# PJLab-ADG/OpenPCSeg

Measured on AMD Instinct MI355X. Metric: LiDAR frames/sec training MinkUNet-34 SemanticKITTI, higher is better.
Workload: dtype f32; 1 GPU; MinkUNet-34 cr1.0 train step, 12 x 120k-pt synthetic SemanticKITTI scans/GPU, fp32; global_batch=12, voxels_per_gpu_batch=1158864, parallelism=dp1, wgrad=fp32

## Files before the change

### include/pcseg_hip.h

```cpp
#ifndef PCSEG_HIP_H_
#define PCSEG_HIP_H_

#include <stddef.h>
#include <stdint.h>

#ifdef __cplusplus
extern "C" {
#endif

#define PCS_OK 0
#define PCS_EINVAL (-1)
#define PCS_EWORKSPACE (-2)
#define PCS_ELAUNCH (-3)
#define PCS_EUNSUPPORTED (-4)

#define PCS_ABI_VERSION 12

int pcs_abi_version(void);
const char *pcs_last_error(void);

int pcs_hash(const int32_t *coords, int64_t n, int64_t *out, void *stream);

int pcs_kernel_hash(const int32_t *coords, int64_t n, const int32_t *offsets, int32_t K,
                    int64_t *out, void *stream);
// ... 233 lines not shown
int pcs_predict_points_f32(const float *logits, int64_t m, int32_t c, const int64_t *inverse, int64_t n,
                           const int64_t *point_offset, const int64_t *row_offset, int32_t n_scenes,
                           const int64_t *labels, float *votes, int64_t *pred, int64_t *hist, int32_t *bad_flag,
                           void *stream);

typedef struct {
  const float *src;
  void *dst;
  int32_t K, A, B;
  int32_t kind;
  int32_t transpose;
  int32_t nctt, nt16, ns;
  int64_t first_block;
} pcs_weight_job;
int64_t pcs_weights_multi_plan(pcs_weight_job *jobs_host, int32_t n_jobs);
int pcs_weights_multi(const pcs_weight_job *jobs_dev, int32_t n_jobs, int64_t total_blocks, void *stream);

int64_t pcs_lovasz_workspace_bytes(int64_t n, int32_t num_class, int32_t has_ignore, int64_t ignore);
int pcs_lovasz_softmax_f32(const float *probas, const int64_t *labels, int64_t n, int32_t num_class, int32_t has_ignore,
                           int64_t ignore, float *loss, float *grad, void *ws, int64_t ws_bytes, void *stream);

void pcs_debug_convh_ws(int32_t mode, int32_t ru, int32_t rs);
void pcs_debug_wgrad_interleave(int32_t mode);

#ifdef __cplusplus
}
#endif
#endif
```

### openpcseg_amd/csrc/conv_wgrad.hip

```cpp
#include "conv_common.h"

using namespace pcs;

namespace {

constexpr int WG_PB = 32;
constexpr int WG_TS = 128 + 16;

struct WgradArgs {
  const float *fa;
  const float *fb;
  const int32_t *pairs;
  const int32_t *koff;
  float *partial;
  int ca, cb, K, a_col, pch;
};

__device__ __forceinline__ void find_split(const int32_t *koff, int K, int pch, int split, int *k_out,
                                           int *beg, int *end) {
  int acc = 0;
  for (int k = 0; k < K; ++k) {
    const int nk = koff[k + 1] - koff[k];
    const int ns = (nk + pch - 1) / pch;
    if (split < acc + ns) {
      const int s = split - acc;
      *k_out = k;
      *beg = koff[k] + s * pch;
      const int e = *beg + pch;
      *end = e < koff[k + 1] ? e : koff[k + 1];
      return;
    }
    acc += ns;
  }
  *k_out = -1; *beg = 0; *end = 0;
}

__device__ __forceinline__ void find_split_wave(const int32_t *koff, int K, int pch, int split, int lane, int *beg,
                                                int *end, int *gsid, int interleave) {
  if (K > 64) {
    int k;
    find_split(koff, K, pch, split, &k, beg, end);
    *gsid = split;
    return;
  }
  const int lo = lane < K ? koff[lane] : 0, hi = lane < K ? koff[lane + 1] : 0;
  const int ns = (hi - lo + pch - 1) / pch;
  int incl = ns;
  for (int o = 1; o < 64; o <<= 1) {
    const int t = __shfl_up(incl, o, 64);
    if (lane >= o) incl += t;
  }
  int src, sidx;
  if (!interleave) {
    const unsigned long long hit = __ballot(split >= incl - ns && split < incl);
    if (!hit) { *beg = 0; *end = 0; *gsid = split; return; }
    src = __ffsll((long long)hit) - 1;
    sidx = split - __shfl(incl - ns, src, 64);
  } else {
    const int total = __shfl(incl, 63, 64);
    if (interleave == 2) {
      const int chunk = (total + 7) >> 3;
      split = (split & 7) * chunk + (split >> 3);
    }
    if (split >= total) { *beg = 0; *end = 0; *gsid = 0; return; }
    int rmax = ns;
    for (int o = 32; o > 0; o >>= 1) { const int t = __shfl_xor(rmax, o, 64); rmax = t > rmax ? t : rmax; }
    auto upto = [&](int r) {
      int c = ns > 0 ? (int)(((long long)r * ns) / rmax) + 1 : 0;
      for (int o = 32; o > 0; o >>= 1) c += __shfl_xor(c, o, 64);
      return c;
    };
    int a = 0, b = rmax - 1;
    while (a < b) {
      const int m = (a + b) >> 1;
      if (upto(m) > split) b = m; else a = m + 1;
    }
    const int r = a;
    const int before = r > 0 ? upto(r - 1) : 0;
    const int s_r = ns > 0 ? (int)(((long long)r * ns) / rmax) : -1;
    const int s_p = (ns > 0 && r > 0) ? (int)(((long long)(r - 1) * ns) / rmax) : -1;
    unsigned long long fresh = __ballot(ns > 0 && s_r != s_p);
    int want = split - before;
    while (want > 0) { fresh &= fresh - 1; --want; }
    src = __ffsll((long long)fresh) - 1;
    sidx = __shfl(s_r, src, 64);
  }
  const int b0 = lo + sidx * pch;
  const int e0 = b0 + pch < hi ? b0 + pch : hi;
  *beg = __shfl(b0, src, 64);
  *end = __shfl(e0, src, 64);
  *gsid = __shfl(incl - ns, src, 64) + sidx;
}

__global__ void __launch_bounds__(256) wgrad_kernel(WgradArgs w) {
  __shared__ __attribute__((aligned(16))) float abuf[WG_PB * WG_TS];
  __shared__ __attribute__((aligned(16))) float bbuf[WG_PB * WG_TS];
  __shared__ int ia[WG_PB], ib[WG_PB];
  __shared__ int sh[3];
  const int tid = threadIdx.x, lane = tid & 63, wid = tid >> 6;
  const int a0 = blockIdx.y * 128, b0 = blockIdx.z * 128;
  const int cat = (w.ca - a0) < 128 ? (w.ca - a0) : 128;
  const int cbt = (w.cb - b0) < 128 ? (w.cb - b0) : 128;
  const int ta_n = (cat + 15) / 16, tb_n = (cbt + 15) / 16;
  if (tid == 0) find_split(w.koff, w.K, w.pch, blockIdx.x, &sh[0], &sh[1], &sh[2]);
  __syncthreads();
  const int beg = sh[1], end = sh[2];
  const int wa = wid >> 1, wb = wid & 1;
  f32x4 acc[4][4];
#pragma unroll
  for (int i = 0; i < 4; ++i)
#pragma unroll
    for (int j = 0; j < 4; ++j) acc[i][j] = (f32x4){0, 0, 0, 0};

  const int capad = ta_n * 16, cbpad = tb_n * 16;
  for (int p0 = beg; p0 < end; p0 += WG_PB) {
    const int np = (end - p0) < WG_PB ? (end - p0) : WG_PB;
    __syncthreads();
    if (tid < WG_PB) {
      int2 p = make_int2(-1, -1);
      if (tid < np) p = reinterpret_cast<const int2 *>(w.pairs)[p0 + tid];
      ia[tid] = w.a_col ? p.y : p.x;
      ib[tid] = w.a_col ? p.x : p.y;
    }
    __syncthreads();
    for (int e = tid; e < WG_PB * capad; e += 256) {
      const int r = e / capad, c = e % capad;
      abuf[r * WG_TS + c] = (r < np && c < cat) ? w.fa[(int64_t)ia[r] * w.ca + a0 + c] : 0.f;
// ... 28 lines not shown
        }
      }
    }
  }
  float *out = w.partial + (int64_t)blockIdx.x * w.ca * w.cb;
  const int g = lane >> 4, l15 = lane & 15;
#pragma unroll
  for (int i = 0; i < 4; ++i) {
    const int ta = wa + 2 * i;
    if (ta >= ta_n) continue;
#pragma unroll
    for (int j = 0; j < 4; ++j) {
      const int tb = wb + 2 * j;
      if (tb >= tb_n) continue;
#pragma unroll
      for (int r = 0; r < 4; ++r) {
        const int ra = ta * 16 + g * 4 + r, cbv = tb * 16 + l15;
        if (ra < cat && cbv < cbt) out[(int64_t)(a0 + ra) * w.cb + b0 + cbv] = acc[i][j][r];
      }
    }
  }
}

__global__ void __launch_bounds__(256) wgrad_reduce_kernel(const float *__restrict__ partial,
                                                           const int32_t *__restrict__ koff,
                                                           int K, int pch, int64_t cc,
                                                           float *__restrict__ gW) {
  const int k = blockIdx.y;
  __shared__ int sh[2];
  if (threadIdx.x == 0) {
    int acc = 0;
    for (int q = 0; q < k; ++q) acc += (koff[q + 1] - koff[q] + pch - 1) / pch;
    sh[0] = acc;
    sh[1] = (koff[k + 1] - koff[k] + pch - 1) / pch;
  }
  __syncthreads();
  const int base = sh[0], ns = sh[1];
  for (int64_t e = (int64_t)blockIdx.x * blockDim.x + threadIdx.x; e < cc;
       e += (int64_t)gridDim.x * blockDim.x) {
    float s = 0.f;
    for (int q = 0; q < ns; ++q) s += partial[(int64_t)(base + q) * cc + e];
    gW[(int64_t)k * cc + e] = s;
  }
}

__global__ void __launch_bounds__(256) wgrad_reduce4_kernel(const float *__restrict__ partial,
                                                            const int32_t *__restrict__ koff,
                                                            int K, int pch, int64_t cc,
                                                            float *__restrict__ gW) {
  const int k = blockIdx.y;
  __shared__ int sh[2];
  __shared__ float4 red[16][16];
  if (threadIdx.x < 64) {
    const int lane = threadIdx.x;
    int acc = 0, mine = 0;
    if (K <= 64) {
      const int nsq = lane < K ? (koff[lane + 1] - koff[lane] + pch - 1) / pch : 0;
      int incl = nsq;
      for (int o = 1; o < 64; o <<= 1) {
        const int t = __shfl_up(incl, o, 64);
        if (lane >= o) incl += t;
      }
      acc = __shfl(incl - nsq, k, 64);
      mine = __shfl(nsq, k, 64);
    } else {
      for (int q = 0; q < k; ++q) acc += (koff[q + 1] - koff[q] + pch - 1) / pch;
      mine = (koff[k + 1] - koff[k] + pch - 1) / pch;
    }
    if (lane == 0) { sh[0] = acc; sh[1] = mine; }
  }
  __syncthreads();
  const int base = sh[0], ns = sh[1];
  const int et = threadIdx.x & 15, ql = threadIdx.x >> 4;
  const int64_t e = ((int64_t)blockIdx.x * 16 + et) * 4;
  const bool ok = e < cc;
  const float *p = partial + (int64_t)base * cc + (ok ? e : 0);
  float4 s0 = {0, 0, 0, 0}, s1 = s0, s2 = s0, s3 = s0;
  int q = ql;
  for (; q + 48 < ns; q += 64) {
    const float4 v0 = *reinterpret_cast<const float4 *>(p + (int64_t)q * cc);
    const float4 v1 = *reinterpret_cast<const float4 *>(p + (int64_t)(q + 16) * cc);
    const float4 v2 = *reinterpret_cast<const float4 *>(p + (int64_t)(q + 32) * cc);
    const float4 v3 = *reinterpret_cast<const float4 *>(p + (int64_t)(q + 48) * cc);
    s0.x += v0.x; s0.y += v0.y; s0.z += v0.z; s0.w += v0.w;
    s1.x += v1.x; s1.y += v1.y; s1.z += v1.z; s1.w += v1.w;
    s2.x += v2.x; s2.y += v2.y; s2.z += v2.z; s2.w += v2.w;
    s3.x += v3.x; s3.y += v3.y; s3.z += v3.z; s3.w += v3.w;
  }
  for (; q < ns; q += 16) {
    const float4 v0 = *reinterpret_cast<const float4 *>(p + (int64_t)q * cc);
    s0.x += v0.x; s0.y += v0.y; s0.z += v0.z; s0.w += v0.w;
  }
  s0.x += s1.x + (s2.x + s3.x); s0.y += s1.y + (s2.y + s3.y);
  s0.z += s1.z + (s2.z + s3.z); s0.w += s1.w + (s2.w + s3.w);
  red[ql][et] = s0;
  __syncthreads();
  if (ql == 0 && ok) {
    float4 t = red[0][et];
#pragma unroll
    for (int j = 1; j < 16; ++j) {
      const float4 v = red[j][et];
      t.x += v.x; t.y += v.y; t.z += v.z; t.w += v.w;
    }
    *reinterpret_cast<float4 *>(gW + (int64_t)k * cc + e) = t;
  }
}

struct Wgrad2Args {
  const void *fa;
  const void *fb;
  const int32_t *pairs;
  const int32_t *koff;
  float *partial;
  int ca, cb, K, a_col, pch, nbg;
  int interleave;
};

__host__ __device__ inline int wg_ngroups(int c) { return (c + 63) / 64; }
__host__ __device__ inline int wg_gwidth(int c) {
  const int per = (c + wg_ngroups(c) - 1) / wg_ngroups(c);
  return (per + 15) / 16 * 16;
}

template <int W> struct WVec;
template <> struct WVec<64> { using T = float4; static constexpr int N = 4; };
template <> struct WVec<48> { using T = float3; static constexpr int N = 3; };
template <> struct WVec<32> { using T = float2; static constexpr int N = 2; };
template <> struct WVec<16> { using T = float;  static constexpr int N = 1; };
__device__ __forceinline__ float wcomp(const float4 &v, int i) { return i == 0 ? v.x : (i == 1 ? v.y : (i == 2 ? v.z : v.w)); }
__device__ __forceinline__ float wcomp(const float3 &v, int i) { return i == 0 ? v.x : (i == 1 ? v.y : v.z); }
__device__ __forceinline__ float wcomp(const float2 &v, int i) { return i == 0 ? v.x : v.y; }
__device__ __forceinline__ float wcomp(const float &v, int) { return v; }

template <typename V, int N> __device__ __forceinline__ V wload(Fp32, const void *base, int64_t elem) {
  return *reinterpret_cast<const V *>(reinterpret_cast<const float *>(base) + elem);
}
template <typename V, int N, typename HT> __device__ __forceinline__ V wload(HT, const void *base, int64_t elem) {
  const uint16_t *p = reinterpret_cast<const uint16_t *>(base) + elem;
// ... 90 lines not shown
#else
    acc[0][0][1] += wcomp(b1s.a[0], 0) + wcomp(b1s.a[1], 0) + wcomp(b1s.a[2], 0) + wcomp(b1s.a[3], 0) + wcomp(b1s.b[0], 0) + wcomp(b1s.b[1], 0) + wcomp(b1s.b[2], 0) + wcomp(b1s.b[3], 0);
#endif
    __builtin_amdgcn_sched_barrier(0);
  }
#pragma unroll
  for (int f = 0; f < NA; ++f) {
#pragma unroll
    for (int r = 0; r < 4; ++r) {
      const int row = a0 + NA * (4 * g + r) + f;
      if (row < w.ca && bok) {
        float *d = out + (int64_t)row * w.cb + bc;
#pragma unroll
        for (int h = 0; h < NB; ++h) d[h] = acc[f][h][r];
      }
    }
  }
}

template <typename ET>
__global__ void __launch_bounds__(256, 3) wgrad2_kernel(Wgrad2Args w) {
  const int tid = threadIdx.x, lane = tid & 63, wid = tid >> 6;
  int beg, end, gsid;
  find_split_wave(w.koff, w.K, w.pch, blockIdx.x, lane, &beg, &end, &gsid, w.interleave);
  const int nag = wg_ngroups(w.ca);
  const int nsb = (w.nbg + 1) >> 1;
  const int sa = blockIdx.y / nsb, sb = blockIdx.y - sa * nsb;
  const int ag = 2 * sa + (wid >> 1), bg = 2 * sb + (wid & 1);
  if (beg >= end || ag >= nag || bg >= w.nbg) return;
  const int aw = wg_gwidth(w.ca), bw = wg_gwidth(w.cb);
  float *out = w.partial + (int64_t)gsid * w.ca * w.cb;
  const int a0 = aw * ag, b0 = bw * bg;
#define PCS_WG_CASE(A, B) if (aw == A && bw == B) { wgrad_block<A, B, ET>(w, a0, b0, beg, end, out, lane); return; }
  PCS_WG_CASE(64, 64) PCS_WG_CASE(64, 48) PCS_WG_CASE(64, 32) PCS_WG_CASE(64, 16)
  PCS_WG_CASE(48, 64) PCS_WG_CASE(48, 48) PCS_WG_CASE(48, 32) PCS_WG_CASE(48, 16)
  PCS_WG_CASE(32, 64) PCS_WG_CASE(32, 48) PCS_WG_CASE(32, 32) PCS_WG_CASE(32, 16)
  PCS_WG_CASE(16, 64) PCS_WG_CASE(16, 48) PCS_WG_CASE(16, 32) PCS_WG_CASE(16, 16)
#undef PCS_WG_CASE
}

constexpr int W3_PB = 32;
constexpr int W3_ROW = 128;

typedef __bf16 w3_bf16x2 __attribute__((ext_vector_type(2)));
typedef float w3_f32x2 __attribute__((ext_vector_type(2)));
typedef __bf16 w3_bf16x8 __attribute__((ext_vector_type(8)));
typedef _Float16 w3_f16x8 __attribute__((ext_vector_type(8)));

struct Wgrad3Args {
  const void *fa;
  const void *fb;
  const int32_t *pairs;
  const int32_t *koff;
  float *partial;
  int ca, cb, K, a_col, pch;
  int aw, bw, nag, nbg, nsb;
  int interleave;
  int nsy = 1;
};

template <typename ET> struct W3Mode;
template <> struct W3Mode<Fp32> { static constexpr int PLANES = 3; using MT = Bf16; };
template <> struct W3Mode<Bf16> { static constexpr int PLANES = 1; using MT = Bf16; };
template <> struct W3Mode<Fp16> { static constexpr int PLANES = 1; using MT = Fp16; };

__device__ __forceinline__ f32x4 w3_mfma(Bf16, const uint4 &a, const uint4 &b, f32x4 c) {
  return __builtin_amdgcn_mfma_f32_16x16x32_bf16(__builtin_bit_cast(w3_bf16x8, a), __builtin_bit_cast(w3_bf16x8, b), c, 0, 0, 0);
}
__device__ __forceinline__ f32x4 w3_mfma(Fp16, const uint4 &a, const uint4 &b, f32x4 c) {
  return __builtin_amdgcn_mfma_f32_16x16x32_f16(__builtin_bit_cast(w3_f16x8, a), __builtin_bit_cast(w3_f16x8, b), c, 0, 0, 0);
}

__device__ __forceinline__ void w3_split(float x, float y, uint32_t &hi, uint32_t &mid, uint32_t &lo) {
  const w3_f32x2 v = {x, y};
  const w3_bf16x2 h = __builtin_convertvector(v, w3_bf16x2);
  const w3_f32x2 r1 = v - __builtin_convertvector(h, w3_f32x2);
  const w3_bf16x2 m = __builtin_convertvector(r1, w3_bf16x2);
  const w3_f32x2 r2 = r1 - __builtin_convertvector(m, w3_f32x2);
  const w3_bf16x2 l = __builtin_convertvector(r2, w3_bf16x2);
  hi = __builtin_bit_cast(uint32_t, h); mid = __builtin_bit_cast(uint32_t, m); lo = __builtin_bit_cast(uint32_t, l);
}

template <typename ET, int NA, int NB, int NT = 256, int ROW = W3_ROW>
__global__ void __launch_bounds__(NT, NT == 256 ? (W3Mode<ET>::PLANES == 1 ? 3 : 2) : 4) wgrad3_kernel(Wgrad3Args w) {
  constexpr int PL = W3Mode<ET>::PLANES;
  using MT = typename W3Mode<ET>::MT;
  constexpr bool F32IN = std::is_same<ET, Fp32>::value;
  constexpr int NBUF = PL == 1 ? 2 : 1;
  constexpr int IMG = PL * 2 * W3_PB * ROW;
  __shared__ __attribute__((aligned(16))) uint16_t lds[NBUF * IMG];
  const int tid = threadIdx.x, lane = tid & 63, wid = tid >> 6;
  const int g = lane >> 4, l15 = lane & 15;
  int beg, end, gsid;
  int bx = blockIdx.x, by = blockIdx.y;
  if (w.interleave == 2 && w.nsy > 1) {
    const int slot = bx >> 3;
    by = slot % w.nsy;
    bx = ((slot / w.nsy) << 3) | (bx & 7);
  }
  find_split_wave(w.koff, w.K, w.pch, bx, lane, &beg, &end, &gsid, w.interleave);
  if (beg >= end) return;
  const int sa = by / w.nsb, sb = by - sa * w.nsb;
  const int a_base = 2 * sa * w.aw, b_base = 2 * sb * w.bw;
  const int a_stage = (w.ca - a_base) < 2 * w.aw ? (w.ca - a_base) : 2 * w.aw;
  const int b_stage = (w.cb - b_base) < 2 * w.bw ? (w.cb - b_base) : 2 * w.bw;
  const int ag = 2 * sa + (wid >> 1), bg = 2 * sb + (wid & 1);
  const bool active = ag < w.nag && bg < w.nbg;
  const int aoff = (wid >> 1) * w.aw, boff = (wid & 1) * w.bw;

  f32x4 acc[NA][NB];
#pragma unroll
  for (int i = 0; i < NA; ++i)
#pragma unroll
    for (int j = 0; j < NB; ++j) acc[i][j] = (f32x4){0, 0, 0, 0};

  constexpr int CPP = F32IN ? 4 : 8;
  constexpr int PPR = ROW / CPP;
  constexpr int PIECES = (W3_PB / 2) * PPR / NT;
  static_assert(PIECES >= 1 && (W3_PB / 2) * PPR % NT == 0, "staging items must divide over the threads");
  uint32_t *ldw = reinterpret_cast<uint32_t *>(lds);
  constexpr int IMGW = IMG / 2;
  constexpr int OPW = (W3_PB / 2) * ROW;
  auto wpos = [](int q, int ch) { return q * ROW + ((((ch >> 4) ^ (q >> 2)) & (ROW / 16 - 1)) << 4) + (ch & 15); };
// ... 116 lines not shown
      __syncthreads();
      if (more) stage(0);
      __syncthreads();
    }
  }
  if (!active) return;
  const int a0 = a_base + aoff, b0 = b_base + boff;
  float *out = w.partial + (int64_t)gsid * w.ca * w.cb;
#pragma unroll
  for (int i = 0; i < NA; ++i)
#pragma unroll
    for (int r = 0; r < 4; ++r) {
      const int row = a0 + 16 * i + 4 * g + r;
      if (row < w.ca) {
#pragma unroll
        for (int j = 0; j < NB; ++j) {
          const int col = b0 + 16 * j + l15;
          if (col < w.cb) out[(int64_t)row * w.cb + col] = acc[i][j][r];
        }
      }
    }
}

struct WgradEnv { int wgrad3, thin, target, interleave; };
const WgradEnv &wgrad_env() {
  auto num = [](const char *v, int dflt) { return v ? atoi(v) : dflt; };
  static const WgradEnv env = {num(getenv("PCS_WGRAD3"), 1),
                               num(getenv("PCS_WGRAD3_THIN"), 1),
                               num(getenv("PCS_WGRAD_TARGET"), 0),
                               num(getenv("PCS_WGRAD_INTERLEAVE"), -1)};
  return env;
}

int g_wgrad_interleave = -1;
enum class WgradFamily { generic, wgrad2, wgrad3, wgrad3_thin };
struct WgradPlan { WgradFamily family; int pch, ns, interleave; dim3 grid; };

int wgrad_splits(const int32_t *koff_host, int K, int pch) {
  int64_t ns = 0;
  for (int k = 0; k < K; ++k) ns += ceil_div((int64_t)koff_host[k + 1] - koff_host[k], pch);
  return (int)ns;
}

WgradPlan wgrad_route(const int32_t *koff_host, int K, int ca, int cb, int dtype, bool force_split, bool operands_aligned,
                      int use3 = wgrad_env().wgrad3, bool count = true) {
  const WgradEnv &env = wgrad_env();
  const bool half = dtype != 0;
  const int nag = wg_ngroups(ca), nbg = wg_ngroups(cb);
  WgradPlan p;
  const bool thin = use3 >= 1 && env.thin && half && ca % 16 == 0 && cb % 16 == 0 && ca <= 64 && cb <= 64 && ca >= 32 && cb >= 32 &&
                    operands_aligned;
  const bool vec = (ca % 4 == 0) && (cb % 4 == 0) && operands_aligned;
  const int cgran = half ? 8 : 4;
  const bool want3 = !half ? (use3 == 2 || force_split) : (use3 >= 1 && (use3 == 2 || nag * nbg >= 4));
  p.family = thin ? WgradFamily::wgrad3_thin
                  : (vec && want3 && ca % cgran == 0 && cb % cgran == 0) ? WgradFamily::wgrad3
                                                                         : (vec ? WgradFamily::wgrad2 : WgradFamily::generic);
  const int nbq = (nag * nbg + 3) / 4;
  const int64_t P = koff_host[K] - koff_host[0];
  int64_t target = (env.target > 0 ? env.target : (nbq >= 4 ? (half ? 2048 : 3072) : 1536)) / nbq;
  if (thin) target *= 4;
  if (target < K) target = K;
  p.pch = (int)ceil_div(P > 0 ? P : 1, target);
  p.pch = (int)(ceil_div(p.pch, 32) * 32);
  if (p.pch < 64) p.pch = 64;
  p.ns = count ? wgrad_splits(koff_host, K, p.pch) : 0;
  p.interleave = g_wgrad_interleave >= 0 ? g_wgrad_interleave : (env.interleave >= 0 ? env.interleave : (half ? 2 : 0));
  const unsigned nx = (unsigned)(p.interleave == 2 ? 8 * ((p.ns + 7) / 8) : p.ns), nsy = (unsigned)(((nag + 1) / 2) * ((nbg + 1) / 2));
  if (p.family == WgradFamily::generic) p.grid = dim3((unsigned)p.ns, (unsigned)ceil_div(ca, 128), (unsigned)ceil_div(cb, 128));
  else if (p.family == WgradFamily::wgrad2) p.grid = dim3(nx, nsy);
  else p.grid = p.interleave == 2 ? dim3(nx * nsy, 1u) : dim3((unsigned)p.ns, nsy);
  return p;
}

template <typename Args>
Args wgrad_args(const void *fa, const void *fb, const int32_t *pairs, const int32_t *koff_dev, void *ws, int ca, int cb, int K,
                int a_col, int pch) {
  Args w;
  w.fa = static_cast<decltype(w.fa)>(fa); w.fb = static_cast<decltype(w.fb)>(fb); w.pairs = pairs; w.koff = koff_dev;
  w.partial = reinterpret_cast<float *>(ws);
  w.ca = ca; w.cb = cb; w.K = K; w.a_col = a_col; w.pch = pch;
  return w;
}

template <typename ET, int NT, int ROW>
int launch_wgrad3(const Wgrad3Args &w, dim3 grid, hipStream_t st, const char *what) {
  const int na = w.aw / 16, nb = w.bw / 16;
#define PCS_W3_CASE(A, B) if constexpr (NT == 256 || (A >= 2 && B >= 2)) if (na == A && nb == B) { hipLaunchKernelGGL((wgrad3_kernel<ET, A, B, NT, ROW>), grid, dim3(NT), 0, st, w); return check_launch(what); }
  PCS_W3_CASE(4, 4) PCS_W3_CASE(4, 3) PCS_W3_CASE(4, 2) PCS_W3_CASE(4, 1)
  PCS_W3_CASE(3, 4) PCS_W3_CASE(3, 3) PCS_W3_CASE(3, 2) PCS_W3_CASE(3, 1)
  PCS_W3_CASE(2, 4) PCS_W3_CASE(2, 3) PCS_W3_CASE(2, 2) PCS_W3_CASE(2, 1)
  PCS_W3_CASE(1, 4) PCS_W3_CASE(1, 3) PCS_W3_CASE(1, 2) PCS_W3_CASE(1, 1)
#undef PCS_W3_CASE
  set_error("%s: unreachable", what);
  return PCS_EINVAL;
}

}

extern "C" size_t pcs_conv_wgrad_ws_bytes(const int32_t *koff_host, int32_t K, int32_t ca, int32_t cb) {
  if (!koff_host || K <= 0 || ca <= 0 || cb <= 0) return 0;
  int pch = INT_MAX;
  for (int dtype = 0; dtype <= 2; ++dtype)
    for (int in = 0; in < 4; ++in)
      for (int use3 = 0; use3 <= 2; ++use3) pch = std::min(pch, wgrad_route(koff_host, K, ca, cb, dtype, in & 1, in & 2, use3, false).pch);
  return (size_t)std::max(wgrad_splits(koff_host, K, pch), 1) * ca * cb * sizeof(float);
}

extern "C" void pcs_debug_wgrad_interleave(int32_t mode) { g_wgrad_interleave = mode; }

static int conv_wgrad_any(const void *fa, int32_t ca, const void *fb, int32_t cb, const int32_t *pairs, int32_t a_col,
                          const int32_t *koff_dev, const int32_t *koff_host, int32_t K, float *gW, void *ws, size_t ws_bytes,
                          int dtype, void *stream, bool force_split = false) {
  if (ca <= 0 || cb <= 0 || K <= 0 || !koff_dev || !koff_host || !gW || (a_col != 0 && a_col != 1) || dtype < 0 || dtype > 2) {
    set_error("pcs_conv_wgrad_f32: bad args");
    return PCS_EINVAL;
  }
  hipStream_t st = as_stream(stream);
  const WgradPlan p = wgrad_route(koff_host, K, ca, cb, dtype, force_split, (((uintptr_t)fa | (uintptr_t)fb) & 15) == 0);
  const int64_t cc = (int64_t)ca * cb;
  if (p.ns == 0) {
    if (hipMemsetAsync(gW, 0, (size_t)K * cc * 4, st) != hipSuccess) { set_error("pcs_conv_wgrad_f32: memset failed"); return PCS_ELAUNCH; }
    return PCS_OK;
  }
  if (!fa || !fb || !pairs || !ws) { set_error("pcs_conv_wgrad_f32: null pointer"); return PCS_EINVAL; }
  if (ws_bytes < (size_t)p.ns * cc * 4) { set_error("pcs_conv_wgrad_f32: workspace too small"); return PCS_EWORKSPACE; }
  const bool vec = p.family != WgradFamily::generic;
  if (dtype != 0 && !vec) { set_error("pcs_conv_wgrad_h: half operands need channel counts that are multiples of 4 and 16-byte aligned tensors"); return PCS_EUNSUPPORTED; }
  switch (p.family) {
    case WgradFamily::generic:
      hipLaunchKernelGGL(wgrad_kernel, p.grid, dim3(256), 0, st, wgrad_args<WgradArgs>(fa, fb, pairs, koff_dev, ws, ca, cb, K, a_col, p.pch));
      break;
    case WgradFamily::wgrad2: {
      Wgrad2Args w = wgrad_args<Wgrad2Args>(fa, fb, pairs, koff_dev, ws, ca, cb, K, a_col, p.pch);
      w.nbg = wg_ngroups(cb); w.interleave = p.interleave;
      if (dtype == 0) hipLaunchKernelGGL(wgrad2_kernel<Fp32>, p.grid, dim3(256), 0, st, w);
      else if (dtype == 1) hipLaunchKernelGGL(wgrad2_kernel<Bf16>, p.grid, dim3(256), 0, st, w);
      else hipLaunchKernelGGL(wgrad2_kernel<Fp16>, p.grid, dim3(256), 0, st, w);
      break;
    }
    default: {
      Wgrad3Args w = wgrad_args<Wgrad3Args>(fa, fb, pairs, koff_dev, ws, ca, cb, K, a_col, p.pch);
      w.aw = wg_gwidth(ca); w.bw = wg_gwidth(cb); w.nag = wg_ngroups(ca); w.nbg = wg_ngroups(cb); w.nsb = (w.nbg + 1) / 2;
      w.interleave = p.interleave;
      w.nsy = ((w.nag + 1) / 2) * w.nsb;
      const bool thin = p.family == WgradFamily::wgrad3_thin;
      const char *what = thin ? "pcs_conv_wgrad(wgrad3 thin)" : "pcs_conv_wgrad(wgrad3)";
      const int rc3 = thin ? (dtype == 1 ? launch_wgrad3<Bf16, 64, 64>(w, p.grid, st, what) : launch_wgrad3<Fp16, 64, 64>(w, p.grid, st, what))
                      : dtype == 0 ? launch_wgrad3<Fp32, 256, W3_ROW>(w, p.grid, st, what)
                      : dtype == 1 ? launch_wgrad3<Bf16, 256, W3_ROW>(w, p.grid, st, what) : launch_wgrad3<Fp16, 256, W3_ROW>(w, p.grid, st, what);
      if (rc3) return rc3;
    }
  }
  int rc = check_launch("pcs_conv_wgrad_f32");
  if (rc) return rc;
  if (vec && (((uintptr_t)ws | (uintptr_t)gW) & 15) == 0) {
    hipLaunchKernelGGL(wgrad_reduce4_kernel, dim3((unsigned)ceil_div(cc, 64), K), dim3(256), 0, st,
                       reinterpret_cast<const float *>(ws), koff_dev, (int)K, p.pch, cc, gW);
  } else {
    int gx = (int)ceil_div(cc, 256);
    if (gx > 64) gx = 64;
    hipLaunchKernelGGL(wgrad_reduce_kernel, dim3(gx, K), dim3(256), 0, st,
                       reinterpret_cast<const float *>(ws), koff_dev, (int)K, p.pch, cc, gW);
  }
  return check_launch("pcs_conv_wgrad_f32(reduce)");
}

extern "C" int pcs_conv_wgrad_f32(const float *fa, int32_t ca, const float *fb, int32_t cb,
                                  const int32_t *pairs, int32_t a_col, const int32_t *koff_dev,
                                  const int32_t *koff_host, int32_t K, float *gW, void *ws,
                                  size_t ws_bytes, void *stream) {
  return conv_wgrad_any(fa, ca, fb, cb, pairs, a_col, koff_dev, koff_host, K, gW, ws, ws_bytes, 0, stream);
}

extern "C" int pcs_conv_wgrad_h(const void *fa, int32_t ca, const void *fb, int32_t cb,
                                const int32_t *pairs, int32_t a_col, const int32_t *koff_dev,
                                const int32_t *koff_host, int32_t K, float *gW, void *ws,
                                size_t ws_bytes, int32_t dtype, void *stream) {
  if (dtype != 1 && dtype != 2) { set_error("pcs_conv_wgrad_h: dtype must be 1 (bf16) or 2 (fp16)"); return PCS_EINVAL; }
  return conv_wgrad_any(fa, ca, fb, cb, pairs, a_col, koff_dev, koff_host, K, gW, ws, ws_bytes, dtype, stream);
}

extern "C" int pcs_conv_wgrad_f32_bf16x3(const float *fa, int32_t ca, const float *fb, int32_t cb,
                                         const int32_t *pairs, int32_t a_col, const int32_t *koff_dev,
                                         const int32_t *koff_host, int32_t K, float *gW, void *ws,
                                         size_t ws_bytes, void *stream) {
// ... 4 lines not shown
```

### openpcseg_amd/native.py

```python
import ctypes
import os
from ctypes import c_char_p, c_double, c_float, c_int32, c_int64, c_size_t, c_void_p

import torch

_LIB_PATH = os.environ.get("PCS_LIB_PATH") or os.path.join(os.path.dirname(os.path.abspath(__file__)), "lib",
                                                          "libpcseg_hip.so")

_P = c_void_p
SIGNATURES = {
    "pcs_abi_version": (c_int32, []),
    "pcs_last_error": (c_char_p, []),
    "pcs_hash": (c_int32, [_P, c_int64, _P, _P]),
    "pcs_kernel_hash": (c_int32, [_P, c_int64, _P, c_int32, _P, _P]),
    "pcs_hashtable_capacity": (c_int64, [c_int64]),
    "pcs_hashtable_bytes": (c_size_t, [c_int64]),
    "pcs_hashtable_build": (c_int32, [_P, c_int64, _P, c_int64, _P]),
    "pcs_hashtable_query": (c_int32, [_P, c_int64, _P, c_int64, _P, _P]),
    "pcs_count": (c_int32, [_P, c_int64, _P, c_int64, _P]),
    "pcs_voxelize_fwd_f32": (c_int32, [_P, _P, _P, c_int64, c_int64, c_int32, _P, _P]),
    "pcs_voxelize_fwd_csr_f32": (c_int32, [_P, _P, _P, _P, c_int64, c_int32, _P, _P]),
    "pcs_voxelize_bwd_f32": (c_int32, [_P, _P, _P, c_int64, c_int32, _P, _P]),
    "pcs_devoxelize_fwd_f32": (c_int32, [_P, _P, _P, c_int64, c_int32, _P, _P]),
    "pcs_devoxelize_bwd_f32": (c_int32, [_P, _P, _P, c_int64, c_int64, c_int32, _P, _P]),
# ... 82 lines not shown
    "pcs_conv_gather_gemm_h_ex": (c_int32, [_P, c_int64, c_int32, _P, c_int32, c_int32, _P, c_int32, _P, c_int32, c_int64,
                                            _P, _P, _P, c_int32, _P, _P, _P]),
    "pcs_conv_x3_applies": (c_int32, [c_int32, c_int32, c_int32]),
    "pcs_conv_x3_column_tiles": (c_int32, [c_int32]),
    "pcs_conv_x3_emits_bn_partials": (c_int32, [c_int32, c_int32, c_int32, c_int32]),
    "pcs_conv_prepared_weights_x3_bytes": (c_size_t, [c_int32, c_int32, c_int32]),
    "pcs_conv_prepare_weights_x3": (c_int32, [_P, c_int32, c_int32, c_int32, c_int32, _P, _P]),
    "pcs_conv_gather_gemm_f32_bf16x3": (c_int32, [_P, c_int64, c_int32, _P, c_int32, c_int32, _P, c_int32, _P, c_int32, c_int64,
                                                  _P, _P, _P, _P, _P]),
    "pcs_conv_wgrad_f32_bf16x3": (c_int32, [_P, c_int32, _P, c_int32, _P, c_int32, _P, _P, c_int32, _P,
                                            _P, c_size_t, _P]),
    "pcs_conv_wgrad_h": (c_int32, [_P, c_int32, _P, c_int32, _P, c_int32, _P, _P, c_int32, _P, _P, c_size_t, c_int32, _P]),
    "pcs_unique_emit": (c_int32, [_P, _P, _P, _P, c_int64, _P, _P, _P, _P]),
    "pcs_cylinder_partition_f32": (c_int32, [_P, c_int64, c_int32, _P, _P, _P, _P, _P, _P, _P]),
    "pcs_voxel_label_vote": (c_int32, [_P, _P, c_int64, c_int64, c_int32, c_int64, _P, _P, _P, _P]),
    "pcs_rows_argmax_gather_f32": (c_int32, [_P, c_int64, c_int32, _P, c_int64, _P, _P]),
    "pcs_predict_points_f32": (c_int32, [_P, c_int64, c_int32, _P, c_int64, _P, _P, c_int32, _P, _P, _P, _P, _P, _P]),
    "pcs_weights_multi_plan": (c_int64, [_P, c_int32]),
    "pcs_weights_multi": (c_int32, [_P, c_int32, c_int64, _P]),
    "pcs_lovasz_workspace_bytes": (c_int64, [c_int64, c_int32, c_int32, c_int64]),
    "pcs_lovasz_softmax_f32": (c_int32, [_P, _P, c_int64, c_int32, c_int32, c_int64, _P, _P, _P, c_int64, _P]),
    "pcs_debug_convh_ws": (None, [c_int32, c_int32, c_int32]),
    "pcs_debug_wgrad_interleave": (None, [c_int32]),
    "pcs_debug_pointvoxel_h_inflight": (None, [c_int32]),
}

class _WeightJob(ctypes.Structure):
    _fields_ = [("src", c_void_p), ("dst", c_void_p), ("K", c_int32), ("A", c_int32), ("B", c_int32), ("kind", c_int32),
                ("transpose", c_int32), ("nctt", c_int32), ("nt16", c_int32), ("ns", c_int32), ("first_block", c_int64)]


ABI_VERSION = 12
_lib = None


def lib_path():
    return _LIB_PATH


def load_library():
    global _lib
    if _lib is not None:
        return _lib
    if not os.path.exists(_LIB_PATH):
        raise RuntimeError(
            "openpcseg_amd: %s is missing -- build it with `python -m openpcseg_amd.build` "
# ... 1090 lines not shown
```

Measured before the change: 106.4 frames/s.

## Apportion wgrad split-K chunks per kernel offset to fill whole occupancy waves

New measurement: 106.3 frames/s (median of 2 runs). Within noise of the previous version (-0.1%).

```diff
diff --git a/include/pcseg_hip.h b/include/pcseg_hip.h
--- a/include/pcseg_hip.h
+++ b/include/pcseg_hip.h
@@ -279,6 +279,9 @@
 
 void pcs_debug_convh_ws(int32_t mode, int32_t ru, int32_t rs);
 void pcs_debug_wgrad_interleave(int32_t mode);
+void pcs_debug_wgrad_plan_mode(int32_t mode);
+int32_t pcs_debug_wgrad_plan(const int32_t *koff_host, int32_t K, int32_t ca, int32_t cb, int32_t dtype, int32_t flags,
+                             int32_t *info, int32_t *chunks, int32_t cap);
 
 #ifdef __cplusplus
 }
diff --git a/openpcseg_amd/csrc/conv_wgrad.hip b/openpcseg_amd/csrc/conv_wgrad.hip
--- a/openpcseg_amd/csrc/conv_wgrad.hip
+++ b/openpcseg_amd/csrc/conv_wgrad.hip
@@ -1,4 +1,7 @@
 #include "conv_common.h"
+
+#include <algorithm>
+#include <atomic>
 
 using namespace pcs;
 
@@ -6,6 +9,35 @@
 
 constexpr int WG_PB = 32;
 constexpr int WG_TS = 128 + 16;
+
+constexpr int WG_KTAB = 64;
+struct WgradSplits {
+  int pch, fit;
+  int nsk[WG_KTAB];
+};
+
+template <typename Tab> __host__ __device__ inline int wg_count(const WgradSplits &sp, Tab nsk, int k, int n) {
+  return sp.fit ? nsk[k] : (n + sp.pch - 1) / sp.pch;
+}
+using WgTable = const int *;
+template <typename Args> __device__ __forceinline__ WgTable wg_table() {
+  const char *args = (const char *)__builtin_amdgcn_kernarg_segment_ptr();
+  return reinterpret_cast<WgTable>(args + offsetof(Args, sp) + offsetof(WgradSplits, nsk));
+}
+__host__ __device__ inline void wg_chunk(const WgradSplits &sp, int lo, int hi, int ns, int s, int *beg, int *end) {
+  const unsigned n = (unsigned)(hi - lo);
+  unsigned b, e;
+  if (sp.fit) {
+    const unsigned nb = (n + 31u) >> 5, q = nb / (unsigned)ns, big = (unsigned)ns - (nb - q * (unsigned)ns), s0 = (unsigned)s, s1 = s0 + 1u;
+    b = 32u * (s0 * q + (s0 > big ? s0 - big : 0u));
+    e = 32u * (s1 * q + (s1 > big ? s1 - big : 0u));
+  } else {
+    b = (unsigned)s * (unsigned)sp.pch;
+    e = b + (unsigned)sp.pch;
+  }
+  *beg = lo + (int)b;
+  *end = lo + (int)(e < n ? e : n);
+}
 
 struct WgradArgs {
   const float *fa;
@@ -13,21 +45,19 @@
   const int32_t *pairs;
   const int32_t *koff;
   float *partial;
-  int ca, cb, K, a_col, pch;
+  int ca, cb, K, a_col;
+  WgradSplits sp;
 };
 
-__device__ __forceinline__ void find_split(const int32_t *koff, int K, int pch, int split, int *k_out,
+__device__ __forceinline__ void find_split(const int32_t *koff, int K, const WgradSplits &sp, WgTable tab, int split, int *k_out,
                                            int *beg, int *end) {
   int acc = 0;
   for (int k = 0; k < K; ++k) {
     const int nk = koff[k + 1] - koff[k];
-    const int ns = (nk + pch - 1) / pch;
+    const int ns = wg_count(sp, tab, k, nk);
     if (split < acc + ns) {
-      const int s = split - acc;
       *k_out = k;
-      *beg = koff[k] + s * pch;
-      const int e = *beg + pch;
-      *end = e < koff[k + 1] ? e : koff[k + 1];
+      wg_chunk(sp, koff[k], koff[k + 1], ns, split - acc, beg, end);
       return;
     }
     acc += ns;
@@ -35,16 +65,16 @@
   *k_out = -1; *beg = 0; *end = 0;
 }
 
-__device__ __forceinline__ void find_split_wave(const int32_t *koff, int K, int pch, int split, int lane, int *beg,
+__device__ __forceinline__ void find_split_wave(const int32_t *koff, int K, const WgradSplits &sp, WgTable tab, int split, int lane, int *beg,
                                                 int *end, int *gsid, int interleave) {
   if (K > 64) {
     int k;
-    find_split(koff, K, pch, split, &k, beg, end);
+    find_split(koff, K, sp, tab, split, &k, beg, end);
     *gsid = split;
     return;
   }
   const int lo = lane < K ? koff[lane] : 0, hi = lane < K ? koff[lane + 1] : 0;
-  const int ns = (hi - lo + pch - 1) / pch;
+  const int ns = wg_count(sp, tab, lane, hi - lo);
   int incl = ns;
   for (int o = 1; o < 64; o <<= 1) {
     const int t = __shfl_up(incl, o, 64);
@@ -85,8 +115,8 @@
     src = __ffsll((long long)fresh) - 1;
     sidx = __shfl(s_r, src, 64);
   }
-  const int b0 = lo + sidx * pch;
-  const int e0 = b0 + pch < hi ? b0 + pch : hi;
+  int b0 = 0, e0 = 0;
+  if (ns > 0) wg_chunk(sp, lo, hi, ns, sidx < ns ? sidx : 0, &b0, &e0);
   *beg = __shfl(b0, src, 64);
   *end = __shfl(e0, src, 64);
   *gsid = __shfl(incl - ns, src, 64) + sidx;
@@ -102,7 +132,7 @@
   const int cat = (w.ca - a0) < 128 ? (w.ca - a0) : 128;
   const int cbt = (w.cb - b0) < 128 ? (w.cb - b0) : 128;
   const int ta_n = (cat + 15) / 16, tb_n = (cbt + 15) / 16;
-  if (tid == 0) find_split(w.koff, w.K, w.pch, blockIdx.x, &sh[0], &sh[1], &sh[2]);
+  if (tid == 0) find_split(w.koff, w.K, w.sp, wg_table<WgradArgs>(), blockIdx.x, &sh[0], &sh[1], &sh[2]);
   __syncthreads();
   const int beg = sh[1], end = sh[2];
   const int wa = wid >> 1, wb = wid & 1;
@@ -177,17 +207,29 @@
   }
 }
 
-__global__ void __launch_bounds__(256) wgrad_reduce_kernel(const float *__restrict__ partial,
-                                                           const int32_t *__restrict__ koff,
-                                                           int K, int pch, int64_t cc,
-                                                           float *__restrict__ gW) {
+struct WgradReduceArgs {
+  const float *partial;
+  const int32_t *koff;
+  float *gW;
+  int64_t cc;
+  int K;
+  WgradSplits sp;
+};
+
+__global__ void __launch_bounds__(256) wgrad_reduce_kernel(WgradReduceArgs w) {
+  const float *__restrict__ partial = w.partial;
+  const int32_t *__restrict__ koff = w.koff;
+  float *__restrict__ gW = w.gW;
+  const int64_t cc = w.cc;
+  const WgradSplits &sp = w.sp;
+  const WgTable tab = wg_table<WgradReduceArgs>();
   const int k = blockIdx.y;
   __shared__ int sh[2];
   if (threadIdx.x == 0) {
     int acc = 0;
-    for (int q = 0; q < k; ++q) acc += (koff[q + 1] - koff[q] + pch - 1) / pch;
+    for (int q = 0; q < k; ++q) acc += wg_count(sp, tab, q, koff[q + 1] - koff[q]);
     sh[0] = acc;
-    sh[1] = (koff[k + 1] - koff[k] + pch - 1) / pch;
+    sh[1] = wg_count(sp, tab, k, koff[k + 1] - koff[k]);
   }
   __syncthreads();
   const int base = sh[0], ns = sh[1];
@@ -199,10 +241,14 @@
   }
 }
 
-__global__ void __launch_bounds__(256) wgrad_reduce4_kernel(const float *__restrict__ partial,
-                                                            const int32_t *__restrict__ koff,
-                                                            int K, int pch, int64_t cc,
-                                                            float *__restrict__ gW) {
+__global__ void __launch_bounds__(256) wgrad_reduce4_kernel(WgradReduceArgs w) {
+  const float *__restrict__ partial = w.partial;
+  const int32_t *__restrict__ koff = w.koff;
+  float *__restrict__ gW = w.gW;
+  const int64_t cc = w.cc;
+  const int K = w.K;
+  const WgradSplits &sp = w.sp;
+  const WgTable tab = wg_table<WgradReduceArgs>();
   const int k = blockIdx.y;
   __shared__ int sh[2];
   __shared__ float4 red[16][16];
@@ -210,7 +256,7 @@
     const int lane = threadIdx.x;
     int acc = 0, mine = 0;
     if (K <= 64) {
-      const int nsq = lane < K ? (koff[lane + 1] - koff[lane] + pch - 1) / pch : 0;
+      const int nsq = lane < K ? wg_count(sp, tab, lane, koff[lane + 1] - koff[lane]) : 0;
       int incl = nsq;
       for (int o = 1; o < 64; o <<= 1) {
         const int t = __shfl_up(incl, o, 64);
@@ -219,8 +265,8 @@
       acc = __shfl(incl - nsq, k, 64);
       mine = __shfl(nsq, k, 64);
     } else {
-      for (int q = 0; q < k; ++q) acc += (koff[q + 1] - koff[q] + pch - 1) / pch;
-      mine = (koff[k + 1] - koff[k] + pch - 1) / pch;
+      for (int q = 0; q < k; ++q) acc += wg_count(sp, tab, q, koff[q + 1] - koff[q]);
+      mine = wg_count(sp, tab, k, koff[k + 1] - koff[k]);
     }
     if (lane == 0) { sh[0] = acc; sh[1] = mine; }
   }
@@ -267,8 +313,9 @@
   const int32_t *pairs;
   const int32_t *koff;
   float *partial;
-  int ca, cb, K, a_col, pch, nbg;
+  int ca, cb, K, a_col, nbg;
   int interleave;
+  WgradSplits sp;
 };
 
 __host__ __device__ inline int wg_ngroups(int c) { return (c + 63) / 64; }
@@ -405,7 +452,7 @@
 __global__ void __launch_bounds__(256, 3) wgrad2_kernel(Wgrad2Args w) {
   const int tid = threadIdx.x, lane = tid & 63, wid = tid >> 6;
   int beg, end, gsid;
-  find_split_wave(w.koff, w.K, w.pch, blockIdx.x, lane, &beg, &end, &gsid, w.interleave);
+  find_split_wave(w.koff, w.K, w.sp, wg_table<Wgrad2Args>(), blockIdx.x, lane, &beg, &end, &gsid, w.interleave);
   const int nag = wg_ngroups(w.ca);
   const int nsb = (w.nbg + 1) >> 1;
   const int sa = blockIdx.y / nsb, sb = blockIdx.y - sa * nsb;
@@ -436,10 +483,11 @@
   const int32_t *pairs;
   const int32_t *koff;
   float *partial;
-  int ca, cb, K, a_col, pch;
+  int ca, cb, K, a_col;
   int aw, bw, nag, nbg, nsb;
   int interleave;
   int nsy = 1;
+  WgradSplits sp;
 };
 
 template <typename ET> struct W3Mode;
@@ -481,7 +529,7 @@
     by = slot % w.nsy;
     bx = ((slot / w.nsy) << 3) | (bx & 7);
   }
-  find_split_wave(w.koff, w.K, w.pch, bx, lane, &beg, &end, &gsid, w.interleave);
+  find_split_wave(w.koff, w.K, w.sp, wg_table<Wgrad3Args>(), bx, lane, &beg, &end, &gsid, w.interleave);
   if (beg >= end) return;
   const int sa = by / w.nsb, sb = by - sa * w.nsb;
   const int a_base = 2 * sa * w.aw, b_base = 2 * sb * w.bw;
@@ -644,24 +692,113 @@
     }
 }
 
-struct WgradEnv { int wgrad3, thin, target, interleave; };
+struct WgradEnv { int wgrad3, thin, target, interleave, plan; };
 const WgradEnv &wgrad_env() {
   auto num = [](const char *v, int dflt) { return v ? atoi(v) : dflt; };
   static const WgradEnv env = {num(getenv("PCS_WGRAD3"), 1),
                                num(getenv("PCS_WGRAD3_THIN"), 1),
                                num(getenv("PCS_WGRAD_TARGET"), 0),
-                               num(getenv("PCS_WGRAD_INTERLEAVE"), -1)};
+                               num(getenv("PCS_WGRAD_INTERLEAVE"), -1),
+                               num(getenv("PCS_WGRAD_PLAN"), 1)};
   return env;
 }
 
 int g_wgrad_interleave = -1;
+int g_wgrad_plan = -1;
 enum class WgradFamily { generic, wgrad2, wgrad3, wgrad3_thin };
-struct WgradPlan { WgradFamily family; int pch, ns, interleave; dim3 grid; };
+struct WgradPlan { WgradFamily family; WgradSplits sp; int ns, interleave, nsy, rounds, slots; dim3 grid; };
 
 int wgrad_splits(const int32_t *koff_host, int K, int pch) {
   int64_t ns = 0;
   for (int k = 0; k < K; ++k) ns += ceil_div((int64_t)koff_host[k + 1] - koff_host[k], pch);
   return (int)ns;
+}
+
+template <typename ET, int NT, int ROW>
+const void *wgrad3_instance(int na, int nb) {
+#define PCS_W3_CASE(A, B) if constexpr (NT == 256 || (A >= 2 && B >= 2)) if (na == A && nb == B) return reinterpret_cast<const void *>(&wgrad3_kernel<ET, A, B, NT, ROW>);
+  PCS_W3_CASE(4, 4) PCS_W3_CASE(4, 3) PCS_W3_CASE(4, 2) PCS_W3_CASE(4, 1)
+  PCS_W3_CASE(3, 4) PCS_W3_CASE(3, 3) PCS_W3_CASE(3, 2) PCS_W3_CASE(3, 1)
+  PCS_W3_CASE(2, 4) PCS_W3_CASE(2, 3) PCS_W3_CASE(2, 2) PCS_W3_CASE(2, 1)
+  PCS_W3_CASE(1, 4) PCS_W3_CASE(1, 3) PCS_W3_CASE(1, 2) PCS_W3_CASE(1, 1)
+#undef PCS_W3_CASE
+  return nullptr;
+}
+
+const void *wgrad_instance(WgradFamily f, int dtype, int na, int nb) {
+  switch (f) {
+    case WgradFamily::generic: return reinterpret_cast<const void *>(&wgrad_kernel);
+    case WgradFamily::wgrad2:
+      return dtype == 0 ? reinterpret_cast<const void *>(&wgrad2_kernel<Fp32>)
+                        : dtype == 1 ? reinterpret_cast<const void *>(&wgrad2_kernel<Bf16>) : reinterpret_cast<const void *>(&wgrad2_kernel<Fp16>);
+    case WgradFamily::wgrad3:
+      return dtype == 0 ? wgrad3_instance<Fp32, 256, W3_ROW>(na, nb)
+                        : dtype == 1 ? wgrad3_instance<Bf16, 256, W3_ROW>(na, nb) : wgrad3_instance<Fp16, 256, W3_ROW>(na, nb);
+    default: return dtype == 1 ? wgrad3_instance<Bf16, 64, 64>(na, nb) : dtype == 2 ? wgrad3_instance<Fp16, 64, 64>(na, nb) : nullptr;
+  }
+}
+
+int wgrad_slots(WgradFamily f, int dtype, int na, int nb) {
+  static std::atomic<int> cache[4][3][5][5];
+  std::atomic<int> &slot = cache[(int)f][dtype][f == WgradFamily::wgrad3 || f == WgradFamily::wgrad3_thin ? na : 0]
+                                [f == WgradFamily::wgrad3 || f == WgradFamily::wgrad3_thin ? nb : 0];
+  int s = slot.load(std::memory_order_relaxed);
+  if (s > 0) return s;
+  const bool thin = f == WgradFamily::wgrad3_thin;
+  int per_cu = thin ? 4 * 4 : (f == WgradFamily::wgrad3 && dtype == 0) || f == WgradFamily::generic ? 2 : 3, cus = 256, dev = 0, v = 0;
+  const void *fn = wgrad_instance(f, dtype, na, nb);
+  if (fn && hipGetDevice(&dev) == hipSuccess) {
+    if (hipOccupancyMaxActiveBlocksPerMultiprocessor(&v, fn, thin ? 64 : 256, 0) == hipSuccess && v > 0) per_cu = v;
+    if (hipDeviceGetAttribute(&v, hipDeviceAttributeMultiprocessorCount, dev) == hipSuccess && v > 0) cus = v;
+  } else {
+    (void)hipGetLastError();
+  }
+  s = per_cu * cus;
+  slot.store(s, std::memory_order_relaxed);
+  return s;
+}
+
+int wgrad_apportion(const int32_t *koff_host, int K, int64_t total, int *nsk) {
+  int64_t n[WG_KTAB], cap[WG_KTAB], pairs = 0, budget = total;
+  bool open[WG_KTAB];
+  int nopen = 0;
+  for (int k = 0; k < K; ++k) {
+    n[k] = (int64_t)koff_host[k + 1] - koff_host[k];
+    cap[k] = n[k] >= 128 ? n[k] / 64 : 1;
+    nsk[k] = 0;
+    open[k] = n[k] > 0;
+    if (open[k]) { pairs += n[k]; ++nopen; }
+  }
+  while (nopen > 0) {
+    bool fixed = false;
+    for (int k = 0; k < K; ++k)
+      if (open[k] && budget * n[k] < pairs) { nsk[k] = 1; open[k] = false; fixed = true; }
+    if (!fixed)
+      for (int k = 0; k < K; ++k)
+        if (open[k] && budget * n[k] >= cap[k] * pairs) { nsk[k] = (int)cap[k]; open[k] = false; fixed = true; }
+    if (!fixed) break;
+    pairs = 0; budget = total; nopen = 0;
+    for (int k = 0; k < K; ++k) {
+      if (open[k]) { pairs += n[k]; ++nopen; }
+      budget -= nsk[k];
+    }
+  }
+  int64_t sum = 0;
+  if (nopen > 0) {
+    int order[WG_KTAB], m = 0;
+    int64_t rem[WG_KTAB], left = budget;
+    for (int k = 0; k < K; ++k)
+      if (open[k]) {
+        nsk[k] = (int)(budget * n[k] / pairs);
+        rem[k] = budget * n[k] % pairs;
+        left -= nsk[k];
+        order[m++] = k;
+      }
+    std::stable_sort(order, order + m, [&](int x, int y) { return rem[x] > rem[y]; });
+    for (int i = 0; i < m && left > 0; ++i, --left) ++nsk[order[i]];
+  }
+  for (int k = 0; k < K; ++k) sum += nsk[k];
+  return (int)sum;
 }
 
 WgradPlan wgrad_route(const int32_t *koff_host, int K, int ca, int cb, int dtype, bool force_split, bool operands_aligned,
@@ -678,17 +815,40 @@
   p.family = thin ? WgradFamily::wgrad3_thin
                   : (vec && want3 && ca % cgran == 0 && cb % cgran == 0) ? WgradFamily::wgrad3
                                                                          : (vec ? WgradFamily::wgrad2 : WgradFamily::generic);
+  p.interleave = g_wgrad_interleave >= 0 ? g_wgrad_interleave : (env.interleave >= 0 ? env.interleave : (half ? 2 : 0));
   const int nbq = (nag * nbg + 3) / 4;
+  p.nsy = p.family == WgradFamily::generic ? (int)(ceil_div(ca, 128) * ceil_div(cb, 128)) : thin ? 1 : ((nag + 1) / 2) * ((nbg + 1) / 2);
   const int64_t P = koff_host[K] - koff_host[0];
-  int64_t target = (env.target > 0 ? env.target : (nbq >= 4 ? (half ? 2048 : 3072) : 1536)) / nbq;
-  if (thin) target *= 4;
-  if (target < K) target = K;
-  p.pch = (int)ceil_div(P > 0 ? P : 1, target);
-  p.pch = (int)(ceil_div(p.pch, 32) * 32);
-  if (p.pch < 64) p.pch = 64;
-  p.ns = count ? wgrad_splits(koff_host, K, p.pch) : 0;
-  p.interleave = g_wgrad_interleave >= 0 ? g_wgrad_interleave : (env.interleave >= 0 ? env.interleave : (half ? 2 : 0));
-  const unsigned nx = (unsigned)(p.interleave == 2 ? 8 * ((p.ns + 7) / 8) : p.ns), nsy = (unsigned)(((nag + 1) / 2) * ((nbg + 1) / 2));
+  const int64_t target_wg = (env.target > 0 ? env.target : (nbq >= 4 ? (half ? 2048 : 3072) : 1536)) * (thin ? 4 : 1);
+  const int mode = g_wgrad_plan >= 0 ? g_wgrad_plan : env.plan;
+  p.sp.fit = K <= WG_KTAB && (mode >= 2 || (mode == 1 && !thin));
+  p.rounds = 0;
+  p.slots = 0;
+  for (int k = 0; k < WG_KTAB; ++k) p.sp.nsk[k] = 0;
+  if (!p.sp.fit) {
+    int64_t target = target_wg / (thin ? 4 : 1) / nbq * (thin ? 4 : 1);
+    if (target < K) target = K;
+    p.sp.pch = (int)ceil_div(P > 0 ? P : 1, target);
+    p.sp.pch = (int)(ceil_div(p.sp.pch, 32) * 32);
+    if (p.sp.pch < 64) p.sp.pch = 64;
+    p.ns = count ? wgrad_splits(koff_host, K, p.sp.pch) : 0;
+  } else {
+    const int np = p.family == WgradFamily::wgrad3 || thin ? wg_gwidth(ca) / 16 : 0, nq = np ? wg_gwidth(cb) / 16 : 0;
+    p.slots = wgrad_slots(p.family, dtype, np, nq);
+    p.rounds = (int)std::max<int64_t>(1, (target_wg + p.slots / 2) / p.slots);
+    int live = 0;
+    for (int k = 0; k < K; ++k) live += koff_host[k + 1] > koff_host[k];
+    auto total_of = [&](int r) {
+      const int64_t t = (int64_t)r * p.slots / p.nsy;
+      return p.interleave == 2 ? t & ~(int64_t)7 : t;
+    };
+    while (total_of(p.rounds) < live) ++p.rounds;
+    const int64_t total = total_of(p.rounds);
+    p.sp.pch = (int)(ceil_div(ceil_div(P > 0 ? P : 1, total), 32) * 32);
+    p.ns = count ? wgrad_apportion(koff_host, K, total, p.sp.nsk) : (int)std::min<int64_t>(total, P / 64 + live);
+    if (live == 0) p.rounds = 0;
+  }
+  const unsigned nx = (unsigned)(p.interleave == 2 ? 8 * ((p.ns + 7) / 8) : p.ns), nsy = (unsigned)p.nsy;
   if (p.family == WgradFamily::generic) p.grid = dim3((unsigned)p.ns, (unsigned)ceil_div(ca, 128), (unsigned)ceil_div(cb, 128));
   else if (p.family == WgradFamily::wgrad2) p.grid = dim3(nx, nsy);
   else p.grid = p.interleave == 2 ? dim3(nx * nsy, 1u) : dim3((unsigned)p.ns, nsy);
@@ -697,39 +857,57 @@
 
 template <typename Args>
 Args wgrad_args(const void *fa, const void *fb, const int32_t *pairs, const int32_t *koff_dev, void *ws, int ca, int cb, int K,
-                int a_col, int pch) {
+                int a_col, const WgradSplits &sp) {
   Args w;
   w.fa = static_cast<decltype(w.fa)>(fa); w.fb = static_cast<decltype(w.fb)>(fb); w.pairs = pairs; w.koff = koff_dev;
   w.partial = reinterpret_cast<float *>(ws);
-  w.ca = ca; w.cb = cb; w.K = K; w.a_col = a_col; w.pch = pch;
+  w.ca = ca; w.cb = cb; w.K = K; w.a_col = a_col; w.sp = sp;
   return w;
 }
 
 template <typename ET, int NT, int ROW>
-int launch_wgrad3(const Wgrad3Args &w, dim3 grid, hipStream_t st, const char *what) {
-  const int na = w.aw / 16, nb = w.bw / 16;
-#define PCS_W3_CASE(A, B) if constexpr (NT == 256 || (A >= 2 && B >= 2)) if (na == A && nb == B) { hipLaunchKernelGGL((wgrad3_kernel<ET, A, B, NT, ROW>), grid, dim3(NT), 0, st, w); return check_launch(what); }
-  PCS_W3_CASE(4, 4) PCS_W3_CASE(4, 3) PCS_W3_CASE(4, 2) PCS_W3_CASE(4, 1)
-  PCS_W3_CASE(3, 4) PCS_W3_CASE(3, 3) PCS_W3_CASE(3, 2) PCS_W3_CASE(3, 1)
-  PCS_W3_CASE(2, 4) PCS_W3_CASE(2, 3) PCS_W3_CASE(2, 2) PCS_W3_CASE(2, 1)
-  PCS_W3_CASE(1, 4) PCS_W3_CASE(1, 3) PCS_W3_CASE(1, 2) PCS_W3_CASE(1, 1)
-#undef PCS_W3_CASE
-  set_error("%s: unreachable", what);
-  return PCS_EINVAL;
+int launch_wgrad3(Wgrad3Args w, dim3 grid, hipStream_t st, const char *what) {
+  const void *fn = wgrad3_instance<ET, NT, ROW>(w.aw / 16, w.bw / 16);
+  if (!fn) { set_error("%s: unreachable", what); return PCS_EINVAL; }
+  void *args[] = {&w};
+  if (hipLaunchKernel(fn, grid, dim3(NT), args, 0, st) != hipSuccess) { (void)hipGetLastError(); set_error("%s: launch failed", what); return PCS_ELAUNCH; }
+  return check_launch(what);
 }
 
 }
 
 extern "C" size_t pcs_conv_wgrad_ws_bytes(const int32_t *koff_host, int32_t K, int32_t ca, int32_t cb) {
   if (!koff_host || K <= 0 || ca <= 0 || cb <= 0) return 0;
-  int pch = INT_MAX;
+  int pch = INT_MAX, ns = 1;
   for (int dtype = 0; dtype <= 2; ++dtype)
     for (int in = 0; in < 4; ++in)
-      for (int use3 = 0; use3 <= 2; ++use3) pch = std::min(pch, wgrad_route(koff_host, K, ca, cb, dtype, in & 1, in & 2, use3, false).pch);
-  return (size_t)std::max(wgrad_splits(koff_host, K, pch), 1) * ca * cb * sizeof(float);
+      for (int use3 = 0; use3 <= 2; ++use3) {
+        const WgradPlan p = wgrad_route(koff_host, K, ca, cb, dtype, in & 1, in & 2, use3, false);
+        if (p.sp.fit) ns = std::max(ns, p.ns);
+        else pch = std::min(pch, p.sp.pch);
+      }
+  if (pch != INT_MAX) ns = std::max(ns, wgrad_splits(koff_host, K, pch));
+  return (size_t)ns * ca * cb * sizeof(float);
+}
+
+extern "C" int32_t pcs_debug_wgrad_plan(const int32_t *koff_host, int32_t K, int32_t ca, int32_t cb, int32_t dtype, int32_t flags,
+                                        int32_t *info, int32_t *chunks, int32_t cap) {
+  if (!koff_host || K <= 0 || ca <= 0 || cb <= 0 || dtype < 0 || dtype > 2 || !info) { set_error("pcs_debug_wgrad_plan: bad args"); return -1; }
+  const WgradPlan p = wgrad_route(koff_host, K, ca, cb, dtype, flags & 1, flags & 2);
+  const int32_t head[12] = {(int32_t)p.family, p.sp.fit, p.ns, p.nsy, p.rounds, p.slots, p.interleave, (int32_t)p.grid.x, (int32_t)p.grid.y,
+                            (int32_t)p.grid.z, p.sp.pch, 0};
+  for (int i = 0; i < 16; ++i) info[i] = i < 12 ? head[i] : 0;
+  for (int k = 0; k < WG_KTAB; ++k) info[16 + k] = p.sp.nsk[k];
+  int i = 0;
+  for (int k = 0; k < K && chunks; ++k) {
+    const int ns = wg_count(p.sp, p.sp.nsk, k < WG_KTAB ? k : 0, koff_host[k + 1] - koff_host[k]);
+    for (int s = 0; s < ns && i < cap; ++s, ++i) wg_chunk(p.sp, koff_host[k], koff_host[k + 1], ns, s, &chunks[2 * i], &chunks[2 * i + 1]);
+  }
+  return p.ns;
 }
 
 extern "C" void pcs_debug_wgrad_interleave(int32_t mode) { g_wgrad_interleave = mode; }
+extern "C" void pcs_debug_wgrad_plan_mode(int32_t mode) { g_wgrad_plan = mode; }
 
 static int conv_wgrad_any(const void *fa, int32_t ca, const void *fb, int32_t cb, const int32_t *pairs, int32_t a_col,
                           const int32_t *koff_dev, const int32_t *koff_host, int32_t K, float *gW, void *ws, size_t ws_bytes,
@@ -751,10 +929,10 @@
   if (dtype != 0 && !vec) { set_error("pcs_conv_wgrad_h: half operands need channel counts that are multiples of 4 and 16-byte aligned tensors"); return PCS_EUNSUPPORTED; }
   switch (p.family) {
     case WgradFamily::generic:
-      hipLaunchKernelGGL(wgrad_kernel, p.grid, dim3(256), 0, st, wgrad_args<WgradArgs>(fa, fb, pairs, koff_dev, ws, ca, cb, K, a_col, p.pch));
+      hipLaunchKernelGGL(wgrad_kernel, p.grid, dim3(256), 0, st, wgrad_args<WgradArgs>(fa, fb, pairs, koff_dev, ws, ca, cb, K, a_col, p.sp));
       break;
     case WgradFamily::wgrad2: {
-      Wgrad2Args w = wgrad_args<Wgrad2Args>(fa, fb, pairs, koff_dev, ws, ca, cb, K, a_col, p.pch);
+      Wgrad2Args w = wgrad_args<Wgrad2Args>(fa, fb, pairs, koff_dev, ws, ca, cb, K, a_col, p.sp);
       w.nbg = wg_ngroups(cb); w.interleave = p.interleave;
       if (dtype == 0) hipLaunchKernelGGL(wgrad2_kernel<Fp32>, p.grid, dim3(256), 0, st, w);
       else if (dtype == 1) hipLaunchKernelGGL(wgrad2_kernel<Bf16>, p.grid, dim3(256), 0, st, w);
@@ -762,10 +940,10 @@
       break;
     }
     default: {
-      Wgrad3Args w = wgrad_args<Wgrad3Args>(fa, fb, pairs, koff_dev, ws, ca, cb, K, a_col, p.pch);
+      Wgrad3Args w = wgrad_args<Wgrad3Args>(fa, fb, pairs, koff_dev, ws, ca, cb, K, a_col, p.sp);
       w.aw = wg_gwidth(ca); w.bw = wg_gwidth(cb); w.nag = wg_ngroups(ca); w.nbg = wg_ngroups(cb); w.nsb = (w.nbg + 1) / 2;
       w.interleave = p.interleave;
-      w.nsy = ((w.nag + 1) / 2) * w.nsb;
+      w.nsy = p.nsy;
       const bool thin = p.family == WgradFamily::wgrad3_thin;
       const char *what = thin ? "pcs_conv_wgrad(wgrad3 thin)" : "pcs_conv_wgrad(wgrad3)";
       const int rc3 = thin ? (dtype == 1 ? launch_wgrad3<Bf16, 64, 64>(w, p.grid, st, what) : launch_wgrad3<Fp16, 64, 64>(w, p.grid, st, what))
@@ -776,14 +954,13 @@
   }
   int rc = check_launch("pcs_conv_wgrad_f32");
   if (rc) return rc;
+  const WgradReduceArgs ra = {reinterpret_cast<const float *>(ws), koff_dev, gW, cc, (int)K, p.sp};
   if (vec && (((uintptr_t)ws | (uintptr_t)gW) & 15) == 0) {
-    hipLaunchKernelGGL(wgrad_reduce4_kernel, dim3((unsigned)ceil_div(cc, 64), K), dim3(256), 0, st,
-                       reinterpret_cast<const float *>(ws), koff_dev, (int)K, p.pch, cc, gW);
+    hipLaunchKernelGGL(wgrad_reduce4_kernel, dim3((unsigned)ceil_div(cc, 64), K), dim3(256), 0, st, ra);
   } else {
     int gx = (int)ceil_div(cc, 256);
     if (gx > 64) gx = 64;
-    hipLaunchKernelGGL(wgrad_reduce_kernel, dim3(gx, K), dim3(256), 0, st,
-                       reinterpret_cast<const float *>(ws), koff_dev, (int)K, p.pch, cc, gW);
+    hipLaunchKernelGGL(wgrad_reduce_kernel, dim3(gx, K), dim3(256), 0, st, ra);
   }
   return check_launch("pcs_conv_wgrad_f32(reduce)");
 }
diff --git a/openpcseg_amd/native.py b/openpcseg_amd/native.py
--- a/openpcseg_amd/native.py
+++ b/openpcseg_amd/native.py
@@ -128,6 +128,8 @@
     "pcs_lovasz_softmax_f32": (c_int32, [_P, _P, c_int64, c_int32, c_int32, c_int64, _P, _P, _P, c_int64, _P]),
     "pcs_debug_convh_ws": (None, [c_int32, c_int32, c_int32]),
     "pcs_debug_wgrad_interleave": (None, [c_int32]),
+    "pcs_debug_wgrad_plan_mode": (None, [c_int32]),
+    "pcs_debug_wgrad_plan": (c_int32, [_P, c_int32, c_int32, c_int32, c_int32, c_int32, _P, _P, c_int32]),
     "pcs_debug_pointvoxel_h_inflight": (None, [c_int32]),
 }
 
```
